# lh3/ksw2

Measured on AMD Instinct MI355X. Metric: GCUPS (DP cells/s) + pairs/s at fixed (qlen,tlen,band), higher is better.
Workload: dtype int16x2 (packed, two alignments per lane); 1 GPU; 10k: 49152 pairs/step/GPU, qlen=10000 tlen=10000 band=500 zdrop=400 extz2 affine score-only; setup_priming_batches=0, parallelism=pairs sharded over 1 GPU(s), one process per GPU, no collective in the data path

## Files before the change

### ksw2_amd/csrc/ksw2_host_plan.c

```c
#include "ksw2_host_int.h"


__thread char g_err[512];
__thread int g_no_defer;
static __thread int g_probe_tasks;
size_t thread_cached_device_bytes(void);

const char *ksw2amd_last_error(void) { return g_err; }
const char *ksw2amd_backend(void) { return k2a_shim_backend(); }
int ksw2amd_device_count(void) { return k2a_shim_device_count(); }


void ksw2amd_release_cache(void);

static const char *const g_env_name[ENV_COUNT] = {
#define X(n) "KSW2AMD_" #n,
	K2A_ENV_LIST
#undef X
};
__thread void *g_plan_stream;
__thread int g_latency_plan;
const char *g_env[ENV_COUNT];
volatile int g_env_ready;
static int g_env_gen;
// ... 835 lines not shown
				e_->tf = (uint32_t)p->h_pairs[i].tlen_full;
			}
		for (b = 0, k = 0; b < NB; ++b) {
			const int cnt = bcnt[b], pass = b % NPASS;
			sort_t *g = srt + (bpos[b] - cnt);
			int ntask = 0;
			cls_t *c;
			if (cnt == 0) continue;
			ci = b / NPASS;
			if (!uni) {
			for (i = 1; i < cnt && cmp_cost_desc(&g[i - 1], &g[i]) <= 0; ++i) {}
			if (i < cnt) qsort(g, (size_t)cnt, sizeof(sort_t), cmp_cost_desc);
			}
			c = &p->cls[p->ncls++];
			c->solo = pass == PASS_SOLO;
			c->cfg = c->solo ? 0 : pass ? (pass - 1) % K2A_NPKCFG : ci / 6; c->rb = pass && !c->solo ? ((pass - 1) / K2A_NPKCFG) & 1 : 0;
			c->nomax = !c->solo && pass > 2 * K2A_NPKCFG; c->mode = (ci / 2) % 3; c->generic = ci & 1; c->pk = pass != 0 && !c->solo; c->first = k;
			build_scoring(dual, m, sc->mat, q, e, q2, e2, c->generic, &c->sc);
			if (pkinfo[c->generic].ok > 0) { memcpy(c->sc.cp, pkinfo[c->generic].cp, sizeof(c->sc.cp)); c->sc.pk_smax = pkinfo[c->generic].smax; c->sc.pk_tn1 = pkinfo[c->generic].tn1; c->sc.pk_base = pkinfo[c->generic].base; c->sc.pk_tnc = pkinfo[c->generic].tnc; }
			if (uni) {
				if (!pass || c->solo) { for (i = 0; i < cnt; ++i) p->h_order[k++] = (uint32_t)i; ntask = cnt; }
				else for (i = 0; i < cnt; i += 2, ++ntask) { p->h_order[k++] = (uint32_t)i; p->h_order[k++] = (uint32_t)(i + 1 < cnt ? i + 1 : i); }
			} else
			if (!pass || c->solo) {
				for (i = 0; i < cnt; ++i) p->h_order[k++] = g[i].idx;
				ntask = cnt;
			} else {
				for (i = 0; i < cnt; ++ntask) {
					const uint32_t ia = g[i].idx;
					uint32_t ib = ia;
					if (i + 1 < cnt && g[i + 1].cost == g[i].cost && g[i + 1].tf == g[i].tf) { ib = g[i + 1].idx; i += 2; } else i += 1;
					p->h_order[k++] = ia; p->h_order[k++] = ib;
				}
			}
			c->count = ntask;
			p->ntasks += ntask;
		}
		p->norder = k;
		free(srt); srt = 0;
	}

	if (tlev) tph[4] = now_ms();
	for (k = 0; k < p->ncls; ++k) {
		const cls_t *c = &p->cls[k];
		if (!c->pk || c->cfg != K2A_PKCFG_MP) continue;
		for (i = 0; i < c->count; ++i) {
			K2aPair *da = &p->h_pairs[p->h_order[c->first + 2 * i]], *db = &p->h_pairs[p->h_order[c->first + 2 * i + 1]];
			p->bnd_words = align_up(p->bnd_words, 4);
			da->bnd_off = db->bnd_off = (uint32_t)p->bnd_words;
			p->bnd_words += align_up((size_t)da->qlen * (dual ? 5 : 4) + 16, 4) + K2A_PKMP_WAVES * (size_t)(64 * 16 * 2 * 2);
			if (p->bnd_words > 0xfff00000u) { fail(KSW2AMD_E_PARAM, "plan_create: boundary rows over 16 GiB in one plan%s", 0); goto err; }
		}
	}

	{
		const char *ev = ENV(DEFER);
		const int forced = ev && *ev ? (atoi(ev) != 0) : -1;
		size_t ck_total = 0;
		for (k = 0; k < p->ncls; ++k) {
			cls_t *c = &p->cls[k];
			c->defer = c->pk && !c->solo && c->cfg != K2A_PKCFG_MP && !dual && c->mode == K2A_MODE_SCORE && !c->nomax && !g_no_defer &&
			           (forced < 0 ? k2a_pkcfg_G[c->cfg] == 64 && (k2a_shim_simd_count() > 0 ? 2 * (int64_t)(g_probe_tasks ? g_probe_tasks : c->count) >= 3 * (int64_t)k2a_shim_simd_count()
			                                                                                      : (g_probe_tasks ? g_probe_tasks : c->count) >= 32) : forced);
		}
		if (g_probe_tasks) { free(pk_ok); free(solo_ok); return p; }
		for (lo = 0; lo < 2; ++lo) {
			size_t at = p->tb_bytes;
			for (k = 0; k < p->ncls; ++k) {
				const cls_t *c = &p->cls[k];
				const int G = c->pk ? k2a_pkcfg_G[c->cfg] : 64, C = c->pk ? k2a_pkcfg_C[c->cfg] : 16, NG = 64 / G;
				int t0;
				if (!c->defer) continue;
				at += align_up(4 * K2A_ZLIST_WORDS(c->count), 256);
				for (t0 = 0; t0 < c->count; t0 += NG) {
					uint32_t steps = 0, hs = 0;
					int t;
					size_t bytes;
					for (t = t0; t < imin(c->count, t0 + NG); ++t) {
						const K2aPair *d = &p->h_pairs[p->h_order[c->first + 2 * t]];
						const uint32_t ns = (uint32_t)((d->tlen + C - 1) / C);
						steps = (uint32_t)imax((int)steps, (int)ns - 1 + imin(d->qlen - 1, d->tlen - 1 + d->w) + 1);
						hs = (uint32_t)imax((int)hs, (int)ns);
					}
					bytes = align_up((size_t)steps * 512 + (size_t)NG * hs * 16, 256);
					if (lo) for (t = t0; t < imin(c->count, t0 + NG); ++t) {
						K2aPair *da = &p->h_pairs[p->h_order[c->first + 2 * t]], *db = &p->h_pairs[p->h_order[c->first + 2 * t + 1]];
						da->tb_off = db->tb_off = at; da->bnd_off = db->bnd_off = steps; da->cig_off = db->cig_off = hs;
					}
					at += bytes;
				}
			}
			if (!lo) {
				ck_total = at - p->tb_bytes;
				if (ck_total > ((size_t)1 << 30) && forced < 0) {
					size_t free_b = 0, total_b = 0;
					if (k2a_shim_mem_info(&free_b, &total_b) || ck_total > (free_b + thread_cached_device_bytes()) / 10 * 6) {
						for (k = 0; k < p->ncls; ++k) p->cls[k].defer = 0;
						ck_total = 0;
						break;
					}
				}
				if (ck_total == 0) break;
			} else p->tb_bytes = at;
		}
	}

	for (k = 0; k < p->ncls; ++k) {
		const cls_t *c = &p->cls[k];
		if (c->mode == K2A_MODE_SCORE) continue;
		for (i = 0; i < c->count; ++i) {
			const uint32_t ia = p->h_order[c->first + (c->pk ? 2 * i : i)];
			const uint32_t ib = c->pk ? p->h_order[c->first + 2 * i + 1] : ia;
			K2aPair *da = &p->h_pairs[ia], *db = &p->h_pairs[ib];
			const int G = c->pk ? k2a_pkcfg_G[c->cfg] : k2a_cfg_G[c->cfg], C = c->pk ? k2a_pkcfg_C[c->cfg] : k2a_cfg_C[c->cfg];
			const int nstrips = (da->tlen + C - 1) / C;
			size_t steps = (size_t)(nstrips - 1) + (size_t)imin(da->qlen - 1, da->tlen - 1 + da->w) + 1;
			const size_t wb = c->pk ? (size_t)K2A_PK_TB_BYTES(C, dual) : (size_t)C * (dual ? 8 : 4) / 8;
			if (!c->solo && (c->pk ? c->cfg == K2A_PKCFG_MP : c->cfg == K2A_CFG_MP)) steps = mp_total_steps(G, C, da->qlen, da->tlen, da->w);
			da->tb_off = db->tb_off = p->tb_bytes;
			if (c->solo) {
				const int nds = (da->tlen + 2 * K2A_SOLO_C - 1) / (2 * K2A_SOLO_C);
				p->tb_bytes += align_up(K2A_TB_PADDED((size_t)(2 * (nds - 1) + 2) + (size_t)imin(da->qlen - 1, da->tlen - 1 + da->w)) * 64 * 2 * K2A_SOLO_C, 256);
			} else
			p->tb_bytes += align_up(K2A_TB_PADDED(steps) * G * wb, 256);
			da->cig_off = (uint32_t)p->cig_words;
			p->cig_words += (size_t)da->qlen + da->tlen_full + 2;
			if (ib != ia) { db->cig_off = (uint32_t)p->cig_words; p->cig_words += (size_t)db->qlen + db->tlen_full + 2; }
			if (p->cig_words > 0xfff00000u) { fail(KSW2AMD_E_PARAM, "plan_create: CIGAR scratch over 16 GiB in one plan%s", 0); goto err; }
		}
	}

	for (k = 0; k < p->ncls; ++k) p->cls[k].qd = -1;
	if (su) {
		size_t at = 0;
		const char *te = ENV(STREAM_TIMEOUT_MS);
		const uint64_t ticks = (uint64_t)(te && atoi(te) > 0 ? atoi(te) : 2000) * 100000u;
		for (k = 0; k < p->ncls; ++k) {
			cls_t *c = &p->cls[k];
			if (c->pk && !c->solo && c->cfg != K2A_PKCFG_MP && c->mode == K2A_MODE_SCORE) c->qd = p->nqd++;
		}
		if (p->nqd) {
			p->h_qd = (K2aQueueDesc*)calloc((size_t)p->nqd, sizeof(K2aQueueDesc));
			if (!p->h_qd) { fail(KSW2AMD_E_NOMEM, "plan_create: host allocation failed%s", 0); goto err; }
			for (k = 0; k < p->ncls; ++k) {
				const cls_t *c = &p->cls[k];
				const int NG = c->qd >= 0 ? 64 / k2a_pkcfg_G[c->cfg] : 1, nwt = (c->count + NG - 1) / NG;
				uint32_t *need = p->h_order + p->norder + at;
				int wt, t;
				if (c->qd < 0) continue;
				for (wt = 0; wt < nwt; ++wt) {
					uint32_t nd = 0;
					for (t = wt * NG; t < imin(c->count, (wt + 1) * NG); ++t) {
						const uint32_t na = p->h_half[p->h_order[c->first + 2 * t]], nb = p->h_half[p->h_order[c->first + 2 * t + 1]];
						if (na > nd) nd = na;
						if (nb > nd) nd = nb;
					}
					need[wt] = nd;
				}
				p->h_qd[c->qd].nwt = (uint32_t)nwt; p->h_qd[c->qd].timeout_ticks = ticks;
				p->h_qd[c->qd].unp_fmt = (uint32_t)at;
				at += (size_t)nwt;
			}
			p->need_words = at;
			p->streamed = 1;
		}
	}

// ... 78 lines not shown
		    k2a_shim_event_record(p->up_ev, up)) {
			if (shared_up) pthread_mutex_unlock(&g_shared_issue_mu);
			fail(KSW2AMD_E_NODEVICE, "upload failed: %s", k2a_shim_last_error());
			goto err;
		}
		if (shared_up) pthread_mutex_unlock(&g_shared_issue_mu);
	}
	if (m > 5) for (k = 0; k < p->ncls; ++k) p->cls[k].sc.mat = (const int8_t*)p->d_seq + mat_off + (p->cls[k].generic ? (size_t)m * m : 0);
	free(pk_ok); free(solo_ok);
	p->flat_tail = flat_tmp; flat_tmp = 0;
	free(flat_tmp);
	plan_ready(p);
	if (tlev) { const double t6 = now_ms(); char tmsg[96]; tmsg[0] = 0; if (su) snprintf(tmsg, sizeof(tmsg), "; streamed: %d pieces, %.3f ms in the upload calls so far", su->np, su->issue_ms); fprintf(stderr, "[ksw2_amd] plan_create n=%d: host arrays + arena layout %.3f, copy + classify %.3f, shape parity + demotions %.3f, sequence upload call + task lists %.3f, traceback layout %.3f, uploads + sync %.3f ms%s\n", n, tph[1] - tph[0], tph[2] - tph[1], tph[3] - tph[2], tph[4] - tph[3] , tph[5] - tph[4], t6 - tph[5], tmsg); }
	return p;
err:
	if (p && p->gather) gather_wait(p);
	if ((flat_tmp || su) && p && p->stream_used && p->stream) k2a_shim_stream_sync(p->stream);
	free(srt); free(pk_ok); free(solo_ok); free(flat_tmp);
	ksw2amd_plan_destroy(p);
	return 0;
}

#define K2A_UNI_MIN_PAIRS 2048
void uni_fill_range(const K2aUniform *u, K2aPair *hp, int8_t *h_cls, int32_t *h_flag, uint32_t *h_order, int cls0, int flag0, int beg, int end)
{
	int i;
	for (i = beg; i < end; ++i) {
		K2aPair d = u->tmpl;
		d.qoff = (uint32_t)i * u->stride; d.toff = (uint32_t)i * u->stride + u->qpad;
		if (u->defer) d.tb_off = u->blk_base + (uint64_t)(((uint32_t)i >> 1) / u->ng) * u->blk_bytes;
		hp[i] = d; h_cls[i] = (int8_t)cls0; h_flag[i] = flag0; h_order[i] = (uint32_t)i;
	}
}

static ksw2amd_plan_t *plan_create_uniform(int dual, int scalar, const ksw2amd_scoring_t *sc, int n, const ksw2amd_pair_t *pairs)
{
	ksw2amd_plan_t *t, *p = 0;
	stream_up_t *su = 0;
	K2aUniform *u = 0;
	cls_t c0;
	K2aPair tm;
	int cls0, flag0, k, G, C, NG, nwt, mx, w, wire4;
	size_t pbytes, ppp;
	uint8_t *d_pk = 0;
	const char *ev = ENV(UNIFORM);
	g_err[0] = 0;
	if ((ev && atoi(ev) == 0) || n < K2A_UNI_MIN_PAIRS || (n & 1) || !pairs || !sc || sc->m > 5 || sc->m <= 0 || !sc->mat) return 0;
	if (!(pairs[0].flag & KSW_EZ_SCORE_ONLY) || pairs[0].qlen <= 0 || pairs[0].tlen <= 0 || !pairs[0].query || !pairs[0].target) return 0;
	if (stream_env() == 0 || g_no_defer || g_probe_tasks || 0) return 0;
	g_probe_tasks = n / 2;
	t = plan_create_ex(dual, scalar, sc, 2, pairs, 0, 0);
	g_probe_tasks = 0;
	if (!t) return 0;
	if (t->reject_all || t->ncls != 1 || !t->cls[0].pk || t->cls[0].solo || t->cls[0].cfg == K2A_PKCFG_MP || t->cls[0].mode != K2A_MODE_SCORE || t->cls[0].count != 1) {
		ksw2amd_plan_destroy(t); g_err[0] = 0; return 0;
	}
	c0 = t->cls[0]; tm = t->h_pairs[0]; cls0 = t->h_cls[0]; flag0 = t->h_flag[0];
	p = plan_new("plan_create", n, -1);
	if (!p) { ksw2amd_plan_destroy(t); return 0; }
	p->dual = !!dual; p->m = sc->m; p->scalar = scalar;
	p->src_mat = t->src_mat; t->src_mat = 0;
	p->src_sc = *sc; p->src_sc.mat = p->src_mat;
	ksw2amd_plan_destroy(t);
	p->h_cls[n] = -1; memset(&p->h_pairs[n], 0, sizeof(K2aPair)); p->h_half[n] = 0;
	u = (K2aUniform*)calloc(1, sizeof(*u));
	p->h_order = (uint32_t*)malloc(sizeof(uint32_t) * ((size_t)n + 4));
	if (!u || !p->h_order) { free(u); fail(KSW2AMD_E_NOMEM, "plan_create: host allocation failed%s", 0); goto err; }
	p->uni = u;
	mx = imax(pairs[0].qlen, pairs[0].tlen); w = pairs[0].w; if (w < 0 || w > mx) w = mx;
	p->cells = (int64_t)n * band_cells(pairs[0].qlen, pairs[0].tlen, w);
	u->n = (uint32_t)n; u->ntasks = (uint32_t)(n / 2);
	wire4 = (ENV(WIRE4) && atoi(ENV(WIRE4)) == 0) ? 0 : (ENV(WIRE2) && atoi(ENV(WIRE2)) == 1) ? 2 : 1;
	u->qpad = (uint32_t)align_up((size_t)pairs[0].qlen, 16); u->stride = u->qpad + (uint32_t)align_up((size_t)pairs[0].tlen + 64 + (wire4 == 2 ? K2A_WIRE2_PAD : 0), 16);
	if (wire4 == 2 && u->stride >= (1u << 20)) { wire4 = 1; u->stride = u->qpad + (uint32_t)align_up((size_t)pairs[0].tlen + 64, 16); }
	if ((uint64_t)n * u->stride > 0xfff00000u - 65536u) { g_err[0] = 0; goto na; }
	p->seq_bytes = align_up((size_t)n * u->stride + 65536, 256);
	u->seq_bytes = p->seq_bytes; u->margin = K2A_STREAM_MARGIN;
	tm.cig_off = 0; tm.tb_off = 0; tm.bnd_off = 0; tm.pad = 0;
	G = k2a_pkcfg_G[c0.cfg]; C = k2a_pkcfg_C[c0.cfg]; NG = 64 / G; nwt = (n / 2 + NG - 1) / NG;
	u->ng = (uint32_t)NG;
	p->ncls = 1; p->cls[0] = c0; p->cls[0].first = 0; p->cls[0].count = n / 2; p->cls[0].qd = 0; p->ntasks = n / 2; p->norder = n;
	if (c0.defer) {
		const uint32_t ns = (uint32_t)((tm.tlen + C - 1) / C), steps = ns - 1 + (uint32_t)imin(tm.qlen - 1, tm.tlen - 1 + tm.w) + 1;
		const size_t bytes = align_up((size_t)steps * 512 + (size_t)NG * ns * 16, 256), zl = align_up(4 * K2A_ZLIST_WORDS(n / 2), 256);
		size_t free_b = 0, total_b = 0;
		if (zl + (size_t)nwt * bytes > ((size_t)1 << 30) && !(ENV(DEFER) && *ENV(DEFER)) &&
		    (k2a_shim_mem_info(&free_b, &total_b) || zl + (size_t)nwt * bytes > (free_b + thread_cached_device_bytes()) / 10 * 6)) { g_err[0] = 0; goto na; }
		u->defer = 1; u->blk_base = zl; u->blk_bytes = bytes;
		tm.bnd_off = steps; tm.cig_off = ns;
		p->tb_bytes = zl + (size_t)nwt * bytes;
	}
	u->tmpl = tm;
	p->h_seq = (uint8_t*)cache_get(BUF_HSEQ, (p->seq_bytes >> wire4) + 256, &p->cap[BUF_HSEQ]);
	su = (stream_up_t*)calloc(1, sizeof(*su));
	if (!p->h_seq || !su) { free(su); su = 0; fail(KSW2AMD_E_NOMEM, "pinned staging allocation failed: %s", k2a_shim_last_error()); goto err; }
	p->up_state = su;
	su->t0 = now_ms();
	pthread_mutex_init(&su->mu, 0);
	{
		const char *pk_ = ENV(STREAM_PIECE_KB);
		pbytes = pk_ && atol(pk_) > 0 ? (size_t)atol(pk_) << 10 : p->seq_bytes / 24;
		if (!(pk_ && atol(pk_) > 0)) { if (pbytes < ((size_t)1 << 20)) pbytes = (size_t)1 << 20; if (pbytes > ((size_t)32 << 20)) pbytes = (size_t)32 << 20; }
		if (wire4 && pbytes < ((size_t)K2A_WM_BYTES << wire4)) pbytes = (size_t)K2A_WM_BYTES << wire4;
		if (pbytes * (K2A_MAXPIECES - 1) < p->seq_bytes) pbytes = p->seq_bytes / (K2A_MAXPIECES - 1) + 1;
		ppp = (pbytes + u->stride - 1) / u->stride;
		if (ppp < 1) ppp = 1;
		while (((size_t)n + ppp - 1) / ppp > K2A_MAXPIECES) ++ppp;
	}
	su->np = (int)(((size_t)n + ppp - 1) / ppp);
	for (k = 0; k <= su->np; ++k) {
		const size_t first = (size_t)k * ppp < (size_t)n ? (size_t)k * ppp : (size_t)n;
		su->pfirst[k] = (int)first; su->pb[k] = k < su->np ? first * u->stride : p->seq_bytes;
		u->pb[k] = su->pb[k];
		su->pb[k] >>= wire4;
	}
	su->wire4 = wire4; su->wire_stride = u->stride;
	u->npieces = (uint32_t)su->np;
	su->wm_src = 0;
	{
		extern const uint32_t *k2a_wm_source(void);
		su->wm_src = k2a_wm_source();
	}
	su->up = shared_upload_stream();
	su->up2 = stream_lanes(0) == 2 ? shared_upload_stream2() : 0;
	su->fault = env_flag(ENV(STREAM_FAULT), 0); su->sleep_us = ENV(STREAM_SLEEP_US) ? atoi(ENV(STREAM_SLEEP_US)) : 0;
	su->src = p->h_seq; su->src_bytes = p->seq_bytes >> wire4;
	p->d_seq = (uint8_t*)cache_get(BUF_SEQ, p->seq_bytes, &p->cap[BUF_SEQ]);
	if (wire4) d_pk = (uint8_t*)cache_get(BUF_PK4, p->seq_bytes >> wire4, &p->cap[BUF_PK4]);
	p->d_wm = (uint8_t*)cache_get(BUF_WM, K2A_WM_BYTES + NCLS_ENTRIES * sizeof(K2aQueueDesc), &p->cap[BUF_WM]);
	p->d_pairs = (K2aPair*)cache_get(BUF_PAIRS, sizeof(K2aPair) * ((size_t)n + 1), &p->cap[BUF_PAIRS]);
	p->d_order = (uint32_t*)cache_get(BUF_ORDER, sizeof(uint32_t) * ((size_t)n + (size_t)nwt + 1), &p->cap[BUF_ORDER]);
	p->d_res = (K2aResult*)cache_get(BUF_RES, sizeof(K2aResult) * ((size_t)n + 1), &p->cap[BUF_RES]);
	p->d_tb = p->tb_bytes ? (uint8_t*)cache_get(BUF_TB, p->tb_bytes, &p->cap[BUF_TB]) : 0;
	p->h_meta = (uint8_t*)cache_get(BUF_HMETA, 256, &p->cap[BUF_HMETA]);
	p->h_qd = (K2aQueueDesc*)calloc(1, sizeof(K2aQueueDesc));
	p->wm_ev = k2a_shim_event_create(); p->meta_ev = k2a_shim_event_create(); p->up_ev = k2a_shim_event_create();
	if (!su->wm_src || !su->up || !p->d_seq || !p->d_wm || !p->d_pairs || !p->d_order || !p->d_res || (p->tb_bytes && !p->d_tb) || !p->h_meta || !p->h_qd ||
	    !p->wm_ev || !p->meta_ev || !p->up_ev || (wire4 && !d_pk)) { fail(KSW2AMD_E_NOMEM, "device allocation failed: %s", k2a_shim_last_error()); goto err; }
	su->d_seq = wire4 ? d_pk : p->d_seq; su->d_wm = p->d_wm;
	p->d_pk4 = d_pk;
	p->unscanned = 1; p->npieces = su->np; p->stream = su->up; p->stream_used = 1;
	{
		const char *te = ENV(STREAM_TIMEOUT_MS);
		p->nqd = 1; p->need_words = (size_t)nwt;
		p->h_qd[0].nwt = (uint32_t)nwt; p->h_qd[0].timeout_ticks = (uint64_t)(te && atoi(te) > 0 ? atoi(te) : 2000) * 100000u;
		p->h_qd[0].need = p->d_order + p->norder; p->h_qd[0].wm = (const uint32_t*)p->d_wm;
		if (wire4) {
			p->h_qd[0].unp_src = d_pk; p->h_qd[0].unp_dst = p->d_seq;
			p->h_qd[0].unp_bytes = 2u * (uint32_t)NG * u->stride; p->h_qd[0].unp_total = (uint32_t)n * u->stride;
			p->h_qd[0].unp_fmt = ((uint32_t)wire4 << 30) | u->stride;
		}
		memcpy(p->h_meta, p->h_qd, sizeof(K2aQueueDesc));
	}
	if (k2a_shim_h2d(p->d_wm, (const uint8_t*)su->wm_src + (size_t)K2A_MAXPIECES * K2A_WM_BYTES, K2A_WM_BYTES, su->up) || k2a_shim_event_record(p->wm_ev, su->up) ||
	    k2a_shim_h2d(p->d_wm + K2A_WM_BYTES, p->h_meta, sizeof(K2aQueueDesc), su->up) || k2a_shim_event_record(p->meta_ev, su->up)) {
		fail(KSW2AMD_E_NODEVICE, "upload failed: %s", k2a_shim_last_error()); goto err;
	}
	su->hold = su->np;
	p->streamed = 1;
	{
		extern int gather_start_uniform(ksw2amd_plan_t *p, stream_up_t *su, const ksw2amd_pair_t *pairs, int n, int cls0, int flag0);
		if (gather_start_uniform(p, su, pairs, n, cls0, flag0)) {
			copy_ctx_t cc = { 0 };
			memset(&cc, 0, sizeof(cc));
			cc.h_seq = p->h_seq; cc.hp = p->h_pairs; cc.pairs = pairs; cc.su = su;
			for (k = 0; k < su->np; ++k) {
				extern void copy_or_pack_range(const copy_ctx_t *c, int beg, int end);
// ... 607 lines not shown
```

### ksw2_amd/csrc/ksw2_shim_hip.hip

```cpp
#include <hip/hip_runtime.h>
#include <stdio.h>
#include <string.h>
#include "ksw2_shim.h"
#include "ksw2_lane.h"
#include "ksw2_lane_pk.h"
#include "ksw2_lane_pkmp.h"
#include "ksw2_lane_solo.h"
#include "ksw2_lane_dm.h"
#include "ksw2_lane_extf.h"
#include "ksw2_lane_ssec.h"
#include "ksw2_lane_ssecb.h"
#include "ksw2_lane_extfb.h"
#include "ksw2_lane_ll.h"
#include "ksw2_lane_llchk.h"
#include "ksw2_lane_llsub.h"

#define K2A_WPB 4
#define K2A_TRACE_PPW_MAX 8
static int k2a_trace_ppw(int nwalks)
{
	const int target_waves = 4096;
	int ppw = (nwalks + target_waves - 1) / target_waves;
	return ppw < 1 ? 1 : ppw > K2A_TRACE_PPW_MAX ? K2A_TRACE_PPW_MAX : ppw;
}

static thread_local char g_err[512] = "";

static int set_err(hipError_t e, const char *what)
{
	if (e == hipSuccess) return 0;
	snprintf(g_err, sizeof(g_err), "%s: %s", what, hipGetErrorString(e));
	return -1;
}
#define CHECK(call) do { hipError_t e_ = (call); if (e_ != hipSuccess) return set_err(e_, #call); } while (0)

template<bool UNIFORM>
__device__ __forceinline__ int k2a_wave_id()
{
	return UNIFORM ? __builtin_amdgcn_readfirstlane((int)(threadIdx.x >> 6)) : (int)(threadIdx.x >> 6);
}

#ifndef K2A_STEP_TRIM
#define K2A_STEP_TRIM 1
#endif
#ifndef K2A_INIT_COL0_UNIFORM
#define K2A_INIT_COL0_UNIFORM 1
#endif

template<int G>
__device__ __forceinline__ int k2a_rot1(int v)
{
	constexpr bool BC = K2A_STEP_TRIM != 0;
	if (G == 64) return __builtin_amdgcn_update_dpp(0, v, 0x13C , 0xf, 0xf, BC);
	else if (G == 16) return __builtin_amdgcn_update_dpp(0, v, 0x121 , 0xf, 0xf, BC);
	else {
		const int shifted = __builtin_amdgcn_update_dpp(0, v, 0x111 , 0xf, 0xf, false);
		const int wrapped = __builtin_amdgcn_update_dpp(0, v, 0x129 , 0xf, 0xf, BC);
		return (threadIdx.x & 7) == 0 ? wrapped : shifted;
	}
}

template<int G, int C, bool DUAL, int MODE>
__global__ void __launch_bounds__(64 * K2A_WPB)
k2a_fill_kernel(const K2aScoring sc, const K2aPair *__restrict__ pairs, const uint32_t *__restrict__ order, int ntasks,
                const uint8_t *__restrict__ seq, uint8_t *__restrict__ tb, K2aResult *__restrict__ res)
{
	constexpr int NG = 64 / G;
	typedef K2aLane<G, C, DUAL, MODE> Lane;
	__shared__ K2aBook book[K2A_WPB][NG];
	__shared__ uint32_t tabs[16];
	__shared__ int rowbuf[K2A_WPB][NG][3 * C];
	__shared__ int8_t mtab[K2A_MAXM * K2A_MAXM];
	if (threadIdx.x < 5) { tabs[threadIdx.x] = sc.prof[threadIdx.x]; tabs[8 + threadIdx.x] = (uint32_t)sc.colw[threadIdx.x]; }
	if (sc.m > 5) for (int x = threadIdx.x; x < sc.m * sc.m; x += blockDim.x) mtab[x] = sc.mat[x];
	__syncthreads();

	const int lane = threadIdx.x & 63, wave = k2a_wave_id<true>();
	const int grp = lane / G, gl = lane % G;
	const int task = (blockIdx.x * K2A_WPB + wave) * NG + grp;
	const bool valid = task < ntasks;
	const uint32_t pi = order[valid ? task : 0];
	const K2aPair pr = pairs[pi];

	Lane L;
	L.setup(pr, seq, gl, valid);
	K2aBook *bk = &book[wave][grp];
	if (gl == 0) k2a_book_reset(bk);
	__builtin_amdgcn_wave_barrier();
// ... 141 lines not shown
			if (wall_clock64() - t0 > limit) { __hip_atomic_store(&qd->abort, 1u, __ATOMIC_RELAXED, __HIP_MEMORY_SCOPE_AGENT); return false; }
			if (it < 16) __builtin_amdgcn_s_sleep(16); else __builtin_amdgcn_s_sleep(127);
		}
	}
	__builtin_amdgcn_fence(__ATOMIC_ACQUIRE, "");
	if (qd->unp_bytes) {
		const uint32_t b0 = (uint32_t)wt * qd->unp_bytes, b1 = k2a_span_end(b0, qd->unp_bytes, qd->unp_total);
		if ((qd->unp_fmt >> 30) == 2u) k2a_wire2_task<false>(qd->unp_src, qd->unp_dst, b0, b1, qd->unp_fmt & 0x3fffffffu, (int)(threadIdx.x & 63), 64);
		else {
			const uint32_t *src = (const uint32_t*)(qd->unp_src + (b0 >> 1));
			uint2 *dst = (uint2*)(qd->unp_dst + b0);
			for (uint32_t x = threadIdx.x & 63; x < (b1 - b0) >> 3; x += 64) {
				uint32_t lo, hi;
				k2a_wire4_expand(src[x], lo, hi);
				dst[x] = make_uint2(lo, hi);
			}
		}
		__builtin_amdgcn_fence(__ATOMIC_RELEASE, "agent");
		__builtin_amdgcn_fence(__ATOMIC_ACQUIRE, "agent");
	}
	if ((threadIdx.x & 63) == 0) __hip_atomic_fetch_add(&qd->next, 1u, __ATOMIC_RELAXED, __HIP_MEMORY_SCOPE_AGENT);
	return true;
}

__device__ __forceinline__ void k2a_cptab_fill(const K2aScoring &sc, uint32_t *tab, int lane)
{
	uint32_t v = sc.cp[0];
#pragma unroll
	for (int x = 1; x < 8; ++x) v = lane == x ? sc.cp[x] : v;
	if (lane < 8) tab[lane] = v;
	__builtin_amdgcn_wave_barrier();
}

#ifndef K2A_UNIFORM_ROWMASK
#define K2A_UNIFORM_ROWMASK 1
#endif
#define K2A_SYNC_WN(L) do { (L).wn = __builtin_amdgcn_ballot_w64((L).hasn != 0) != 0; } while (0)
template<int G, int C, bool DUAL, int MODE, bool RB, bool NOMAX, int LDSROW, bool DEFER, bool TN>
__device__ __forceinline__ void
k2a_fill_pk_body(const K2aScoring &sc, const K2aPair *__restrict__ pairs, const uint32_t *__restrict__ order2, int ntasks,
                 const uint8_t *__restrict__ seq, uint8_t *__restrict__ tb, K2aResult *__restrict__ res,
                 int wt, int wave, int lane, int grp, int gl, bool scan_on, uint32_t scan,
                 K2aBook (*book)[64 / G][2], uint32_t *stage_w, uint32_t *lrows, uint32_t (*cptab)[8], uint4 *tbstage, unsigned long long *tbruns)
{
	constexpr int NG = 64 / G;
	typedef K2aLanePk<G, C, DUAL, MODE, RB, NOMAX, LDSROW, DEFER, TN> Lane;
	constexpr int LROW_WORDS = LDSROW == 1 ? K2A_PK_LDSROW_WORDS(C) : LDSROW == 2 ? K2A_PK_LDSCODE_WORDS(C) : 0;
	constexpr int WB = Lane::TBWORDS * 4;
	constexpr bool STAGED = MODE != K2A_MODE_SCORE && (WB == 16 || WB == 32);
	typedef K2aTbStage<STAGED ? WB : 16, K2A_PK_TB_NS(WB, LDSROW)> Stage;

	const int task = wt * NG + grp;
	const bool valid = task < ntasks;
	const uint32_t piA = order2[valid ? 2 * task : 0], piB = order2[valid ? 2 * task + 1 : 0];
	const K2aPair prA = pairs[piA], prB = pairs[piB];
	const int zdropA = prA.zdrop, zdropB = prB.zdrop;
	const bool zseq = NOMAX || RB || __builtin_amdgcn_ballot_w64(valid && (zdropA >= 0 || zdropB >= 0)) != 0;

	k2a_cptab_fill(sc, cptab[wave], lane);
	Lane L;
	L.lrow = &lrows[LDSROW ? wave * LROW_WORDS + lane : 0];
	L.setup(prA, prB, seq, gl, valid, cptab[wave]);
	K2aBook *bkA = &book[wave][grp][0], *bkB = &book[wave][grp][1];
	if (gl == 0) { k2a_book_reset(bkA); k2a_book_reset(bkB); }
	__builtin_amdgcn_wave_barrier();

	const int klast = L.last_step();
	int kmax = __builtin_amdgcn_readfirstlane(klast);
#pragma unroll
	for (int g = 1; g < NG; ++g) kmax = max(kmax, __builtin_amdgcn_readlane(klast, g * G));

	const int ktop1 = valid ? min(prA.qlen - 1, min(C - 1, prA.tlen - 1) + prA.w) : -1;
	int ktop = __builtin_amdgcn_readfirstlane(ktop1);
#pragma unroll
	for (int g = 1; g < NG; ++g) ktop = max(ktop, __builtin_amdgcn_readlane(ktop1, g * G));

	bool gdone = !valid;
	L.load_query_group(0, L.knext == 0 ? L.koff_next : L.koff, L.qwA, L.qwB);
	const size_t tbsteps = (size_t)(klast + 1);
	uint8_t *tbp = tb + prA.tb_off;
	constexpr bool UMASK = K2A_UNIFORM_ROWMASK != 0 && MODE == K2A_MODE_SCORE;
	constexpr bool COL0U = K2A_INIT_COL0_UNIFORM != 0;
	constexpr bool NOSTOP = K2A_STEP_TRIM != 0 && DEFER && NG == 1;
	K2aRowMasks<C> RM;
	RM.reset();
	Stage ST;
	if (STAGED) ST.init(&tbstage[wave * Stage::WORDS], &tbruns[wave * 64], lane, tbp + k2a_tb_word(0, gl, tbsteps, G, WB));
	int kdone = -1;
	const bool ckon = DEFER && __builtin_amdgcn_readfirstlane((int)valid) != 0;
	const size_t ckoff = DEFER ? ((size_t)(uint32_t)__builtin_amdgcn_readfirstlane((int)(uint32_t)(prA.tb_off >> 32)) << 32) | (uint32_t)__builtin_amdgcn_readfirstlane((int)(uint32_t)prA.tb_off) : 0;
	uint2 *ckst = (uint2*)(tb + ckoff) + lane;
	K2aCkHead *ckhd = (K2aCkHead*)(tb + ckoff + (size_t)(uint32_t)__builtin_amdgcn_readfirstlane((int)prA.bnd_off) * K2A_CK_STEP_BYTES) +
	                  (size_t)grp * (uint32_t)__builtin_amdgcn_readfirstlane((int)prA.cig_off);

	bool stop = false;
	for (int kg = 0; kg <= kmax && !stop; kg += 4) {
	uint32_t qpa, qpb;
	L.load_query_group(kg + 4, L.knext <= kg + 4 ? L.koff_next : L.koff, qpa, qpb);
	const int kge = min(kg + 3, kmax);
#pragma nounroll
	for (int k = kg; k <= kge; ++k) {
		k2a_pk hin = (k2a_pk)k2a_rot1<G>((int)L.hout);
		k2a_pk ein = (k2a_pk)k2a_rot1<G>((int)L.eout);
		k2a_pk e2in = DUAL ? (k2a_pk)k2a_rot1<G>((int)L.e2out) : 0u;

		const bool ninit = L.need_init(k);
		const uint64_t initmask = __builtin_amdgcn_ballot_w64(ninit);
		uint64_t col0mask = 0;
		if (initmask != 0) {
			const int bsA = RB ? k2a_rot1<G>(L.baseA) : 0, bsB = RB ? k2a_rot1<G>(L.baseB) : 0;
			if (UMASK || COL0U) col0mask = __builtin_amdgcn_ballot_w64(ninit && L.Snext * C <= L.w);
			if (ninit) {
				L.template do_init<COL0U>(sc, bsA, bsB, 0, COL0U ? col0mask != 0 : true);
				if (k & 3) L.reload_query_group(k);
				if (ckon) { K2aCkHead h; h.baseA = L.baseA; h.baseB = L.baseB; h.hd0 = L.hd0; h.pad = 0; ckhd[L.S] = h; }
			}
			if (TN) K2A_SYNC_WN(L);
		}
		if (UMASK) {
			if (initmask != 0) RM.on_init(initmask, __builtin_amdgcn_ballot_w64(ninit && L.rows_m1 != C - 1), col0mask);
			const int dd = k - L.kd;
			RM.advance(__builtin_amdgcn_ballot_w64((uint32_t)(dd + L.w) <= (uint32_t)(2 * L.w)));
			if (RM.needs_refresh()) {
				const int lo = max(0, dd - L.w), hi = min(L.rows_m1, dd + L.w);
				uint64_t lv[C];
#pragma unroll
				for (int c = 0; c < C; ++c) lv[c] = __builtin_amdgcn_ballot_w64(lo <= c && c <= hi);
				RM.refresh(lv);
			}
		}
		L.hu_prev = hin;
		if (RB) { hin = k2a_pk_add(hin, L.delta); ein = k2a_pk_add(ein, L.delta); if (DUAL) e2in = k2a_pk_add(e2in, L.delta); }
		L.set_qb(Lane::query_pick(L.qwA, L.qwB, k & 3));
		if (k <= ktop) L.top_inputs(sc, k, hin, ein, e2in);

		if (ckon) ckst[(size_t)k * 64] = make_uint2(hin, ein);
		uint32_t tw[Lane::TBWORDS];
		bool live;
		if (UMASK) { K2aRowPredUniform<C> rp(RM, lane); live = L.step_rows(sc, k, hin, ein, e2in, tw, rp); }
		else live = L.step(sc, k, hin, ein, e2in, tw);
		if (STAGED) { ST.put(k, tw, live); ST.step_done(k); kdone = k; }
		else if (MODE != K2A_MODE_SCORE) {
			if (live) {
				uint32_t *dst = (uint32_t*)(tbp + k2a_tb_word((size_t)k, gl, tbsteps, G, Lane::TBWORDS * 4));
#pragma unroll
				for (int x = 0; x + 3 < Lane::TBWORDS; x += 4) *(uint4*)(dst + x) = make_uint4(tw[x], tw[x + 1], tw[x + 2], tw[x + 3]);
				if (Lane::TBWORDS & 2) *(uint2*)(dst + (Lane::TBWORDS & ~3)) = make_uint2(tw[Lane::TBWORDS & ~3], tw[(Lane::TBWORDS & ~3) + 1]);
			}
		}

		const bool nfin = L.need_fin(k);
		const uint64_t finmask = __builtin_amdgcn_ballot_w64(nfin);
		if (finmask != 0) {
			if (UMASK) RM.on_fin(finmask);
			uint32_t *rowbuf = &stage_w[grp * K2A_PK_STAGE(C)];
			if (NOMAX) {
				if (nfin) L.fin_score_only(sc, bkA, bkB);
			} else if (zseq) {
				const bool slow = nfin && !L.fin_fast(sc, bkA, bkB, zdropA, zdropB);
				if (__builtin_amdgcn_ballot_w64(slow) != 0) {
					if (slow) { L.stage_rows(rowbuf); L.do_fin_seq(sc, bkA, bkB, zdropA, zdropB, rowbuf); }
					__builtin_amdgcn_wave_barrier();
					if (!DEFER && bkA->dropped && bkB->dropped) gdone = true;
				}
			} else {
				const bool gfin = ((finmask >> (grp * G)) & (G == 64 ? ~0ull : (1ull << (G & 63)) - 1)) != 0;
				if (nfin) L.stage_rows(rowbuf);
				__builtin_amdgcn_wave_barrier();
				if (gfin) L.fin_local_rows(sc, rowbuf);
				if (nfin) L.end_strip();
				__builtin_amdgcn_wave_barrier();
			}
			if (TN && L.wn) K2A_SYNC_WN(L);
		}
		if (!NOSTOP && zseq && __builtin_amdgcn_ballot_w64(!(gdone || k >= klast)) == 0) { stop = true; break; }
	}
	L.qwA = qpa; L.qwB = qpb;
	}
	if (STAGED) ST.finish(kdone);
	__builtin_amdgcn_wave_barrier();
	if (!zseq) {
		uint32_t *loc = &stage_w[0];
		loc[lane * 5 + 0] = L.lmax; loc[lane * 5 + 1] = L.lmax_t; loc[lane * 5 + 2] = L.lmax_q;
		loc[lane * 5 + 3] = L.lmqe; loc[lane * 5 + 4] = L.lmqe_t;
		__builtin_amdgcn_wave_barrier();
		if (valid && gl == 0) {
			k2a_merge_local(loc + grp * G * 5, G, 0, bkA);
			k2a_merge_local(loc + grp * G * 5, G, 1, bkB);
			bkA->rows = bkB->rows = prA.tlen;
		}
		__builtin_amdgcn_wave_barrier();
		if (valid && prA.tlen == prA.tlen_full && gl == ((prA.tlen_full - 1) % C) % G) {
			const bool reach = prA.tlen_full - 1 + prA.w >= prA.qlen - 1;
			bkA->mte = k2a_pk_lo(L.last_m); bkA->mte_q = k2a_pk_lo(L.last_j);
			bkB->mte = k2a_pk_hi(L.last_m); bkB->mte_q = k2a_pk_hi(L.last_j);
			if (reach) { bkA->score = k2a_pk_lo(L.last_h); bkB->score = k2a_pk_hi(L.last_h); }
		}
		__builtin_amdgcn_wave_barrier();
	}
	const uint64_t sawmask = __builtin_amdgcn_ballot_w64(valid && (scan_on ? (scan & 2u) != 0 : L.saw_wildcard()));
	const bool gsaw = ((sawmask >> (grp * G)) & (G == 64 ? ~0ull : (1ull << (G & 63)) - 1)) != 0;
	if (valid && gl == 0) {
		const K2aBook a = *bkA, b = *bkB;
		k2a_finish(prA, a, &res[piA]);
		if (piB != piA) k2a_finish(prB, b, &res[piB]);
		if (gsaw) { res[piA].pad[0] = 1; res[piB].pad[0] = 1; }
	}
}

template<int G, int C, bool DUAL, int MODE, bool RB, bool NOMAX, int LDSROW = 0, bool DEFER = false, bool QUEUE = false>
__global__ void __launch_bounds__(64 * K2A_WPB, LDSROW == 2 ? (G == 16 ? 4 : 3) : LDSROW ? 2 : 1)
k2a_fill_pk_kernel(const K2aScoring sc, const K2aPair *__restrict__ pairs, const uint32_t *__restrict__ order2, int ntasks,
                   const uint8_t *__restrict__ seq, uint8_t *__restrict__ tb, K2aResult *__restrict__ res, K2aQueueDesc *qd)
{
	constexpr int NG = 64 / G;
	typedef K2aLanePk<G, C, DUAL, MODE, RB, NOMAX, LDSROW, DEFER, false> Lane;
	__shared__ K2aBook book[K2A_WPB][NG][2];
	__shared__ uint32_t stage[K2A_WPB][(NG * K2A_PK_STAGE(C) > 64 * 5) ? NG * K2A_PK_STAGE(C) : 64 * 5];

	const int lane = threadIdx.x & 63, wave = k2a_wave_id<(C <= 8 || LDSROW || (NOMAX && DUAL && MODE != K2A_MODE_SCORE))>();
	const int grp = lane / G, gl = lane % G;
	const int wt = blockIdx.x * K2A_WPB + wave;
	if (DEFER && blockIdx.x == 0 && threadIdx.x == 0) {
		uint32_t *zlist = (uint32_t*)(tb + pairs[order2[0]].tb_off) - K2A_ZLIST_WORDS(ntasks);
		__hip_atomic_store(&zlist[0], 0u, __ATOMIC_RELAXED, __HIP_MEMORY_SCOPE_AGENT);
	}
	if (QUEUE && !k2a_queue_wait(qd, wt)) return;
	constexpr int LROW_WORDS = LDSROW == 1 ? K2A_PK_LDSROW_WORDS(C) : LDSROW == 2 ? K2A_PK_LDSCODE_WORDS(C) : 0;
	__shared__ uint32_t lrows[LDSROW ? K2A_WPB * LROW_WORDS : 1];
	__shared__ uint32_t cptab[K2A_WPB][8];
	constexpr int WB = Lane::TBWORDS * 4;
	constexpr bool STAGED = MODE != K2A_MODE_SCORE && (WB == 16 || WB == 32);
	typedef K2aTbStage<STAGED ? WB : 16, K2A_PK_TB_NS(WB, LDSROW)> Stage;
	__shared__ uint4 tbstage[STAGED ? K2A_WPB * Stage::WORDS : 1];
	__shared__ unsigned long long tbruns[STAGED ? K2A_WPB * 64 : 1];
	const int task = wt * NG + grp;
	uint32_t scan = 0;
	const bool scan_on = sc.pk_tn1 != 0;
	if (scan_on && task < ntasks) {
		const K2aPair pa = pairs[order2[2 * task]], pb = pairs[order2[2 * task + 1]];
		scan = k2a_scan_codes<G>(seq + pa.toff, pa.tlen_full, gl) | k2a_scan_codes<G>(seq + pb.toff, pb.tlen_full, gl);
	}
	{
		const uint64_t m1 = __builtin_amdgcn_ballot_w64((scan & 1u) != 0), m2 = __builtin_amdgcn_ballot_w64((scan & 2u) != 0);
		const uint64_t gm = (G == 64 ? ~0ull : (1ull << (G & 63)) - 1) << (grp * G);
		scan = ((m1 & gm) ? 1u : 0u) | ((m2 & gm) ? 2u : 0u);
		if (m1 != 0 || sc.pk_base != 0)
			k2a_fill_pk_body<G, C, DUAL, MODE, RB, NOMAX, LDSROW, DEFER, true>(sc, pairs, order2, ntasks, seq, tb, res, wt, wave, lane, grp, gl, scan_on, scan, book, stage[wave], lrows, cptab, tbstage, tbruns);
		else
			k2a_fill_pk_body<G, C, DUAL, MODE, RB, NOMAX, LDSROW, DEFER, false>(sc, pairs, order2, ntasks, seq, tb, res, wt, wave, lane, grp, gl, scan_on, scan, book, stage[wave], lrows, cptab, tbstage, tbruns);
	}
}

template<int G, int C, bool RB>
__global__ void __launch_bounds__(64 * K2A_WPB)
k2a_argmax_kernel(const K2aScoring sc, const K2aPair *__restrict__ pairs, const uint32_t *__restrict__ order2, int ntasks,
                  const uint8_t *__restrict__ seq, uint8_t *__restrict__ ck, K2aResult *__restrict__ res, const K2aQueueDesc *qd)
{
	constexpr int NG = 64 / G;
	if (qd && (__hip_atomic_load(&qd->abort, __ATOMIC_RELAXED, __HIP_MEMORY_SCOPE_AGENT) != 0 ||
	           __hip_atomic_load(&qd->next, __ATOMIC_RELAXED, __HIP_MEMORY_SCOPE_AGENT) != qd->nwt)) return;
	typedef K2aLanePk<G, C, false, K2A_MODE_SCORE, RB, false, 0, false, true> Lane;
	const int job = blockIdx.x * (64 * K2A_WPB) + threadIdx.x;
	const int task = job / 3, which = job - 3 * task;
	bool go = task < ntasks;
	const bool live = go;
	const uint32_t piA = order2[go ? 2 * task : 0], piB = order2[go ? 2 * task + 1 : 0];
	const K2aPair prA = pairs[piA], prB = pairs[piB];
	const bool inexA = res[piA].pad[1] != 0, inexB = res[piB].pad[1] != 0;
	int row = -1;
	if (go) {
		if (which == 0) row = res[piA].max_t;
		else if (which == 1) row = piB == piA ? -1 : res[piB].max_t;
		else row = (prA.tlen == prA.tlen_full && !(inexA && inexB)) ? prA.tlen_full - 1 : -1;
	}
	go = go && row >= 0;
	const int S = go ? row / C : 0, grp = task % NG;
	__shared__ uint32_t cptab[K2A_WPB][8];
	k2a_cptab_fill(sc, cptab[threadIdx.x >> 6], (int)(threadIdx.x & 63));
	Lane L;
	L.lrow = 0;
	L.setup(prA, prB, seq, S % G, go, cptab[threadIdx.x >> 6]);
	L.Snext = S;
	L.schedule_next();
	const int kbeg = L.knext;
	const uint8_t *blk = ck + prA.tb_off;
	if (go) L.do_init(sc, 0, 0, (const K2aCkHead*)(blk + (size_t)prA.bnd_off * K2A_CK_STEP_BYTES) + (size_t)grp * prA.cig_off + S);
	K2A_SYNC_WN(L);
	const int n = go ? L.kfin - kbeg + 1 : 0;
	const uint2 *st = (const uint2*)blk + (grp * G + S % G);
	for (int t = 0; __builtin_amdgcn_ballot_w64(t < n) != 0; ++t) {
		if (t < n) {
			const int k = kbeg + t;
			const uint2 in = st[(size_t)k * 64];
			const int jc = min(max(k - L.koff, 0), L.qlen - 1);
			L.set_qb(k2a_pair16(L.qa[jc], L.qbp[jc]));
			uint32_t tw[Lane::TBWORDS];
			L.step(sc, k, in.x, in.y, 0u, tw);
		}
	}
	if (go) {
// ... 2242 lines not shown
```

### ksw2_amd/csrc/ksw2_types.h

```cpp
#ifndef KSW2_TYPES_H_
#define KSW2_TYPES_H_

#include <stdint.h>

#define K2A_NEG      (-0x40000000)
#define K2A_KNONE    0x7fffffff
#define K2A_MAXM     127

#define K2A_F_SCORE_ONLY 0x01
#define K2A_F_EXTZ_ONLY 0x40
#define K2A_F_REV_CIGAR 0x80
#define K2A_F_SPLICE_FOR   0x100
#define K2A_F_SPLICE_REV   0x200
#define K2A_F_SPLICE_FLANK 0x400
#define K2A_F_HAS_JUNC     0x10000000

#define K2A_MODE_SCORE 0
#define K2A_MODE_LEFT  1
#define K2A_MODE_RIGHT 2

#define K2A_TB_PAD 32
#define K2A_TB_PADDED(steps) (((steps) + (K2A_TB_PAD - 1)) / K2A_TB_PAD * K2A_TB_PAD)

#define K2A_NEG16    (-16384)
#define K2A_OFS16    0x4C00
#define K2A_PK_VMAX  (0x7BFF - K2A_OFS16)
#define K2A_PK_SLACK (K2A_OFS16 + K2A_NEG16)
#ifndef K2A_PKMP_T
#define K2A_PKMP_T    64
#endif
#define K2A_PKMP_DEAD (-8192)
#define K2A_PKMP_RMAX_LIMIT 10000
#ifndef K2A_HL_OPEN
#define K2A_HL_OPEN 1
#endif
#define K2A_PK_NIBBLES(C, dual) (!(dual) && (C) == 16)
#define K2A_PK_TB_BYTES(C, dual) (K2A_PK_NIBBLES(C, dual) ? (C) : 2 * (C))

typedef struct K2aScoring {
	int32_t q, e, q2, e2;
	uint32_t prof[5];
	int32_t colw[5];
	uint32_t cp[8];
	int32_t pk_smax;
	int32_t pk_tn1;
	int32_t m;
	const int8_t *mat;
	int32_t pk_base, pk_tnc;
} K2aScoring;

#define K2A_DM_SLOTS_S 8
#define K2A_DM_SLOTS   16
#define K2A_DM_DIAG(K) ((K) * 64 - 64)

typedef struct K2aSplice {
	int32_t q, e, q2, long_thres;
	int32_t m;
	const int8_t *mat;
} K2aSplice;

typedef struct K2aExtf {
	int32_t mch, mis, e;
	int32_t ring;
} K2aExtf;
#define K2A_EXTF_RING_ROWS(span) (((span) + 30) / 4 + 3)

typedef struct K2aSsec {
	int32_t q, e, q2, e2;
	int32_t qe_first;
	int32_t long_thres, long_diff;
	int32_t m, sc_mch, sc_mis, sc_N;
	const int8_t *mat;
} K2aSsec;
#define K2A_SSEC_APPROX      1
#define K2A_SSEC_APPROX_DROP 2
#define K2A_SSEC_GENERIC     4

#define K2A_EXTF_WIN_SPAN(K) (64 * (K) - 109)

typedef struct K2aPair {
	uint32_t qoff, toff;
	int32_t qlen, tlen;
	int32_t tlen_full;
	int32_t w;
	int32_t zdrop, end_bonus, flag;
	uint32_t cig_off;
	uint64_t tb_off;
	uint32_t bnd_off;
	uint32_t pad;
} K2aPair;

typedef struct K2aResult {
	int32_t max, zdropped, max_q, max_t, mqe, mqe_t, mte, mte_q, score, reach_end, n_cigar, rows_done;
	int32_t ti, tj;
	int32_t pad[2];
} K2aResult;

#define K2A_WM_BYTES 65536
#define K2A_WIRE2_ESC 7
#define K2A_WIRE2_SLOT (4 * K2A_WIRE2_ESC)
#define K2A_WIRE2_PAD (4 * K2A_WIRE2_SLOT)

typedef struct K2aQueueDesc {
	uint32_t next;
	uint32_t abort;
	uint32_t nwt;
	uint32_t unp_fmt;
	const uint32_t *need;
	const uint32_t *wm;
	uint64_t timeout_ticks;
	const uint8_t *unp_src;
	uint8_t *unp_dst;
	uint32_t unp_bytes, unp_total;
} K2aQueueDesc;

#define K2A_ZLIST_WORDS(ntasks) ((2 * (size_t)(ntasks) + 16 + 63) & ~(size_t)63)

#define K2A_UNI_MAXPIECES 48
// ... 54 lines not shown
```

Before: 5348 GCUPS.

## Defer per-strip max/zdrop bookkeeping to a post-pass fold over recorded strip rows

In the deferred checkpoint score path with one group per wave, each finished strip now writes its per-row H values and last-column values to a per-task record in global memory, instead of running the max and zdrop bookkeeping inline. After the main DP loop, a wave-wide fold replays these records with a parallel prefix max across strips to recover max, mqe, score and the zdrop stop point. This removes serial bookkeeping from the hot anti-diagonal loop. In exchange it adds extra global writes and checkpoint memory per task, plus a post-pass read.

```diff
diff --git a/ksw2_amd/csrc/ksw2_host_plan.c b/ksw2_amd/csrc/ksw2_host_plan.c
--- a/ksw2_amd/csrc/ksw2_host_plan.c
+++ b/ksw2_amd/csrc/ksw2_host_plan.c
@@ -941,7 +941,7 @@
 						steps = (uint32_t)imax((int)steps, (int)ns - 1 + imin(d->qlen - 1, d->tlen - 1 + d->w) + 1);
 						hs = (uint32_t)imax((int)hs, (int)ns);
 					}
-					bytes = align_up((size_t)steps * 512 + (size_t)NG * hs * 16, 256);
+					bytes = align_up(K2A_CK_BLOCK_BYTES(steps, NG, hs, C), 256);
 					if (lo) for (t = t0; t < imin(c->count, t0 + NG); ++t) {
 						K2aPair *da = &p->h_pairs[p->h_order[c->first + 2 * t]], *db = &p->h_pairs[p->h_order[c->first + 2 * t + 1]];
 						da->tb_off = db->tb_off = at; da->bnd_off = db->bnd_off = steps; da->cig_off = db->cig_off = hs;
@@ -1186,7 +1186,7 @@
 	p->ncls = 1; p->cls[0] = c0; p->cls[0].first = 0; p->cls[0].count = n / 2; p->cls[0].qd = 0; p->ntasks = n / 2; p->norder = n;
 	if (c0.defer) {
 		const uint32_t ns = (uint32_t)((tm.tlen + C - 1) / C), steps = ns - 1 + (uint32_t)imin(tm.qlen - 1, tm.tlen - 1 + tm.w) + 1;
-		const size_t bytes = align_up((size_t)steps * 512 + (size_t)NG * ns * 16, 256), zl = align_up(4 * K2A_ZLIST_WORDS(n / 2), 256);
+		const size_t bytes = align_up(K2A_CK_BLOCK_BYTES(steps, NG, ns, C), 256), zl = align_up(4 * K2A_ZLIST_WORDS(n / 2), 256);
 		size_t free_b = 0, total_b = 0;
 		if (zl + (size_t)nwt * bytes > ((size_t)1 << 30) && !(ENV(DEFER) && *ENV(DEFER)) &&
 		    (k2a_shim_mem_info(&free_b, &total_b) || zl + (size_t)nwt * bytes > (free_b + thread_cached_device_bytes()) / 10 * 6)) { g_err[0] = 0; goto na; }
diff --git a/ksw2_amd/csrc/ksw2_lane_pkfold.h b/ksw2_amd/csrc/ksw2_lane_pkfold.h
--- /dev/null
+++ b/ksw2_amd/csrc/ksw2_lane_pkfold.h
@@ -0,0 +1,131 @@
+#ifndef KSW2_LANE_PKFOLD_H_
+#define KSW2_LANE_PKFOLD_H_
+
+#include "ksw2_lane_pk.h"
+
+#define K2A_PKFOLD_XB_WORDS 256
+
+#if defined(__HIP_DEVICE_COMPILE__)
+#define K2A_FOLD_SYNC() __builtin_amdgcn_wave_barrier()
+#define K2A_FOLD_BALLOT(p, l) __builtin_amdgcn_ballot_w64(p)
+#else
+#define K2A_FOLD_SYNC() do {} while (0)
+#define K2A_FOLD_BALLOT(p, l) ((uint64_t)((p) ? 1u : 0u) << (l))
+#endif
+
+template<int C>
+K2A_FN bool k2a_pkfold_strip_reaches(int s, int qlen, int tlen, int w) { return k2a_min(s * C + C - 1, tlen - 1) + w >= qlen - 1; }
+
+template<int C, int NL>
+K2A_FN void k2a_pkfold_task(const K2aScoring &sc, const uint32_t *rec, const K2aCkHead *hd, int nstrips, int qlen, int tlen, int tlen_full, int w,
+                            int zdropA, int zdropB, K2aBook *bkA, K2aBook *bkB, uint32_t *xb, int lane0)
+{
+	const int hq = k2a_hl_q(sc);
+	const int none = (int)0x80000000;
+	int *xi = (int*)xb;
+#pragma nounroll
+	for (int half = 0; half < 2; ++half) {
+		K2aBook *b = half ? bkB : bkA;
+		const int zdrop = half ? zdropB : zdropA, sh = half ? 16 : 0;
+		int lm[NL], lmt[NL], lq[NL], lqt[NL];
+		for (int x = 0; x < NL; ++x) { lm[x] = lq[x] = none; lmt[x] = lqt[x] = -1; }
+		int carry = b->max;
+		const bool dead = b->dropped != 0 || nstrips <= 0;
+		bool frozen = false;
+		K2A_FOLD_SYNC();
+#pragma nounroll
+		for (int s0 = 0; s0 < nstrips && !dead && !frozen; s0 += 64) {
+			int H[NL][C], hend[NL][C], ent[NL];
+			for (int x = 0; x < NL; ++x) {
+				const int l = lane0 + x, s = s0 + l;
+				int sm = none;
+				if (s < nstrips) {
+					const uint32_t *r = rec + (size_t)s * K2A_CK_REC_WORDS(C);
+					const int base = half ? hd[s].baseB : hd[s].baseA;
+					const bool rs = k2a_pkfold_strip_reaches<C>(s, qlen, tlen, w);
+#pragma unroll
+					for (int c = 0; c < C; ++c) {
+						const int i = s * C + c, unb = base - sc.e * i;
+						H[x][c] = (int)(int16_t)(k2a_ofs_off(r[c]) >> sh) + unb;
+						hend[x][c] = rs ? (int)(int16_t)(k2a_ofs_off(r[C + c]) >> sh) + hq + unb : none;
+						if (i < tlen) sm = k2a_max(sm, H[x][c]);
+					}
+				}
+				xi[l] = sm;
+			}
+			K2A_FOLD_SYNC();
+			int src = 0;
+#pragma nounroll
+			for (int d = 1; d < 64; d <<= 1) {
+				for (int x = 0; x < NL; ++x) {
+					const int l = lane0 + x;
+					int v = xi[src + l];
+					if (l >= d) v = k2a_max(v, xi[src + l - d]);
+					xi[(src ^ 64) + l] = v;
+				}
+				K2A_FOLD_SYNC();
+				src ^= 64;
+			}
+			for (int x = 0; x < NL; ++x) { const int l = lane0 + x; ent[x] = l > 0 ? k2a_max(carry, xi[src + l - 1]) : carry; }
+			carry = k2a_max(carry, xi[src + 63]);
+			K2A_FOLD_SYNC();
+			int tm[NL], tmt[NL], tq[NL], tqt[NL], tmte[NL], tsc[NL], trows[NL];
+			bool fr[NL], hmte[NL], hsc[NL];
+			uint64_t fmask = 0;
+			for (int x = 0; x < NL; ++x) {
+				const int s = s0 + lane0 + x;
+				int m = ent[x];
+				tm[x] = lm[x]; tmt[x] = lmt[x]; tq[x] = lq[x]; tqt[x] = lqt[x]; tmte[x] = tsc[x] = trows[x] = 0;
+				fr[x] = hmte[x] = hsc[x] = false;
+				if (s < nstrips) {
+#pragma unroll
+					for (int c = 0; c < C; ++c) {
+						const int i = s * C + c;
+						if (i < tlen && !fr[x]) {
+							const bool reach = i + w >= qlen - 1;
+							const int h = H[x][c], he = hend[x][c];
+							if (reach && he > tq[x]) { tq[x] = he; tqt[x] = i; }
+							if (i == tlen_full - 1) { tmte[x] = h; hmte[x] = true; }
+							if (h > m) { m = h; tm[x] = h; tmt[x] = i; }
+							else if (zdrop >= 0 && m - h > zdrop) fr[x] = true;
+							if (!fr[x] && i == tlen_full - 1 && reach) { tsc[x] = he; hsc[x] = true; }
+							trows[x] = i + 1;
+						}
+					}
+				}
+				fmask |= K2A_FOLD_BALLOT(fr[x], lane0 + x);
+			}
+			frozen = fmask != 0;
+			const int sfirst = frozen ? s0 + (int)__builtin_ctzll(fmask) : nstrips;
+			for (int x = 0; x < NL; ++x) {
+				const int s = s0 + lane0 + x;
+				if (s < nstrips && s <= sfirst) {
+					lm[x] = tm[x]; lmt[x] = tmt[x]; lq[x] = tq[x]; lqt[x] = tqt[x];
+					if (hmte[x]) { b->mte = tmte[x]; b->mte_q = 0; }
+					if (hsc[x]) b->score = tsc[x];
+					if (fr[x]) { b->dropped = 1; b->inexact = 1; b->rows = trows[x]; }
+				}
+			}
+		}
+		K2A_FOLD_SYNC();
+		for (int x = 0; x < NL; ++x) { const int l = lane0 + x; xi[4 * l] = lm[x]; xi[4 * l + 1] = lmt[x]; xi[4 * l + 2] = lq[x]; xi[4 * l + 3] = lqt[x]; }
+		K2A_FOLD_SYNC();
+		for (int x = 0; x < NL; ++x) {
+			if (lane0 + x == 0 && !dead) {
+				int bm = b->max, bmt = b->max_t, bmq = b->max_q, bq = b->mqe, bqt = b->mqe_t;
+				bool qlane = false;
+#pragma nounroll
+				for (int l = 0; l < 64; ++l) {
+					const int vm = xi[4 * l], vmt = xi[4 * l + 1], vq = xi[4 * l + 2], vqt = xi[4 * l + 3];
+					if (vm != none && vm > bm) { bm = vm; bmt = vmt; bmq = 0; }
+					if (vq != none && (vq > bq || (qlane && vq == bq && vqt < bqt))) { bq = vq; bqt = vqt; qlane = true; }
+				}
+				b->max = bm; b->max_t = bmt; b->max_q = bmq; b->mqe = bq; b->mqe_t = bqt;
+				if (!frozen) b->rows = tlen;
+			}
+		}
+		K2A_FOLD_SYNC();
+	}
+}
+
+#endif
diff --git a/ksw2_amd/csrc/ksw2_shim_hip.hip b/ksw2_amd/csrc/ksw2_shim_hip.hip
--- a/ksw2_amd/csrc/ksw2_shim_hip.hip
+++ b/ksw2_amd/csrc/ksw2_shim_hip.hip
@@ -4,6 +4,7 @@
 #include "ksw2_shim.h"
 #include "ksw2_lane.h"
 #include "ksw2_lane_pk.h"
+#include "ksw2_lane_pkfold.h"
 #include "ksw2_lane_pkmp.h"
 #include "ksw2_lane_solo.h"
 #include "ksw2_lane_dm.h"
@@ -311,6 +312,7 @@
 	constexpr bool UMASK = K2A_UNIFORM_ROWMASK != 0 && MODE == K2A_MODE_SCORE;
 	constexpr bool COL0U = K2A_INIT_COL0_UNIFORM != 0;
 	constexpr bool NOSTOP = K2A_STEP_TRIM != 0 && DEFER && NG == 1;
+	constexpr bool FOLD = K2A_FOLD_AFTER != 0 && DEFER && NG == 1 && !NOMAX && MODE == K2A_MODE_SCORE;
 	K2aRowMasks<C> RM;
 	RM.reset();
 	Stage ST;
@@ -321,6 +323,7 @@
 	uint2 *ckst = (uint2*)(tb + ckoff) + lane;
 	K2aCkHead *ckhd = (K2aCkHead*)(tb + ckoff + (size_t)(uint32_t)__builtin_amdgcn_readfirstlane((int)prA.bnd_off) * K2A_CK_STEP_BYTES) +
 	                  (size_t)grp * (uint32_t)__builtin_amdgcn_readfirstlane((int)prA.cig_off);
+	uint32_t *ckrec = (uint32_t*)(ckhd + (FOLD ? (uint32_t)__builtin_amdgcn_readfirstlane((int)prA.cig_off) : 0u));
 
 	bool stop = false;
 	for (int kg = 0; kg <= kmax && !stop; kg += 4) {
@@ -383,7 +386,18 @@
 		if (finmask != 0) {
 			if (UMASK) RM.on_fin(finmask);
 			uint32_t *rowbuf = &stage_w[grp * K2A_PK_STAGE(C)];
-			if (NOMAX) {
+			if (FOLD) {
+				if (nfin) {
+					uint4 *r4 = (uint4*)(ckrec + (size_t)L.S * K2A_CK_REC_WORDS(C));
+#pragma unroll
+					for (int c = 0; c < C; c += 4) r4[c / 4] = make_uint4(L.rmax(c), L.rmax(c + 1), L.rmax(c + 2), L.rmax(c + 3));
+					if (k2a_pkfold_strip_reaches<C>(L.S, L.qlen, L.tlen, L.w)) {
+#pragma unroll
+						for (int c = 0; c < C; c += 4) r4[(C + c) / 4] = make_uint4(L.hl[c], L.hl[c + 1], L.hl[c + 2], L.hl[c + 3]);
+					}
+					L.end_strip();
+				}
+			} else if (NOMAX) {
 				if (nfin) L.fin_score_only(sc, bkA, bkB);
 			} else if (zseq) {
 				const bool slow = nfin && !L.fin_fast(sc, bkA, bkB, zdropA, zdropB);
@@ -408,7 +422,12 @@
 	}
 	if (STAGED) ST.finish(kdone);
 	__builtin_amdgcn_wave_barrier();
-	if (!zseq) {
+	if (FOLD) {
+		__builtin_amdgcn_fence(__ATOMIC_RELEASE, "workgroup");
+		__builtin_amdgcn_fence(__ATOMIC_ACQUIRE, "workgroup");
+		if (ckon) k2a_pkfold_task<C, 1>(sc, ckrec, ckhd, L.nstrips, L.qlen, L.tlen, L.tlen_full, L.w, zdropA, zdropB, bkA, bkB, stage_w, lane);
+		__builtin_amdgcn_wave_barrier();
+	} else if (!zseq) {
 		uint32_t *loc = &stage_w[0];
 		loc[lane * 5 + 0] = L.lmax; loc[lane * 5 + 1] = L.lmax_t; loc[lane * 5 + 2] = L.lmax_q;
 		loc[lane * 5 + 3] = L.lmqe; loc[lane * 5 + 4] = L.lmqe_t;
@@ -446,6 +465,7 @@
 	typedef K2aLanePk<G, C, DUAL, MODE, RB, NOMAX, LDSROW, DEFER, false> Lane;
 	__shared__ K2aBook book[K2A_WPB][NG][2];
 	__shared__ uint32_t stage[K2A_WPB][(NG * K2A_PK_STAGE(C) > 64 * 5) ? NG * K2A_PK_STAGE(C) : 64 * 5];
+	static_assert(64 * 5 >= K2A_PKFOLD_XB_WORDS, "the fold's exchange buffer is the stage");
 
 	const int lane = threadIdx.x & 63, wave = k2a_wave_id<(C <= 8 || LDSROW || (NOMAX && DUAL && MODE != K2A_MODE_SCORE))>();
 	const int grp = lane / G, gl = lane % G;
diff --git a/ksw2_amd/csrc/ksw2_types.h b/ksw2_amd/csrc/ksw2_types.h
--- a/ksw2_amd/csrc/ksw2_types.h
+++ b/ksw2_amd/csrc/ksw2_types.h
@@ -34,6 +34,12 @@
 #ifndef K2A_HL_OPEN
 #define K2A_HL_OPEN 1
 #endif
+#ifndef K2A_FOLD_AFTER
+#define K2A_FOLD_AFTER 1
+#endif
+#define K2A_CK_REC_WORDS(C) (2 * (C))
+#define K2A_CK_BLOCK_BYTES(steps, NG, hs, C) \
+	((size_t)(steps) * 512 + (size_t)(NG) * (hs) * 16 + ((K2A_FOLD_AFTER) && (NG) == 1 ? (size_t)(hs) * K2A_CK_REC_WORDS(C) * 4 : (size_t)0))
 #define K2A_PK_NIBBLES(C, dual) (!(dual) && (C) == 16)
 #define K2A_PK_TB_BYTES(C, dual) (K2A_PK_NIBBLES(C, dual) ? (C) : 2 * (C))
 
```

Result: faster. 5664 GCUPS, median of 6 (+5.9%).
